# g8a9/multi-modal-emotion

Measured on AMD Instinct MI355X. Metric: utterances/sec fwd+bwd (+clip_grad_norm_+AdamW inside the timed step), TAV (BERT+Wav2Vec2+VideoMAE) b=32, 1/2/4/8 MI355X, higher is better.
Workload: dtype bf16; 1 GPU; tav_nn.py TAV preset B (bert 12 L + wav2vec2 12 L / 768 + videomae 12 L / 768 on 16 frames + fusion 12 L), global batch 32 = 32 per GPU x 1, text 128 tok, audio 80000 samples, video 16x3x224x224 (104 fusion / 1464 encoder tokens), 547.0 GFLOP forward per utterance; global_batch=32, per_gpu_batch=32, parallelism=dp1, weights=random init (seeded), no checkpoints offline, launch=hipGraph replay

## Files before the change

include/tavhip.h:

```cpp
#ifndef TAVHIP_H
#define TAVHIP_H
#include <stdint.h>

#ifdef __cplusplus
extern "C" {
#endif

enum { TAV_F32 = 0, TAV_BF16 = 1, TAV_FP8 = 2  };
enum {
    TAV_ERR_NULL = -1,
    TAV_ERR_SHAPE = -2,
    TAV_ERR_DTYPE = -3,
    TAV_ERR_ALIGN = -4,
    TAV_ERR_NO_RCCL = -5
};

int tav_version(void);
const char* tav_error_string(int code);

typedef struct tav_gemm_nt_args {
    const void* A; const void* B; void* C;
    void* C_pre;
    const float* bias;
    const void* gelu_in;
// ... 20 lines not shown
    float* out;
    float* dbias;
    float* bias_partials;
    int64_t N1, N2;
    int64_t lda, ldb;
    int64_t rows_per_batch, nbatch;
    int64_t a_zb, b_zb;
    int32_t chunk_rows, nsplit;
    int32_t perm_inner, perm_outer;
    int32_t dtype;
    int32_t accumulate;
    float scale;
} tav_gemm_tn_args;
int tav_gemm_tn_splits(int64_t n1, int64_t n2, int64_t rows_per_batch, int64_t nbatch, int32_t* chunk_rows, int32_t* nsplit);
int tav_gemm_tn(const tav_gemm_tn_args* args, void* stream);

typedef struct tav_gemm_tn_problem {
    const void* A; const void* B;
    float* out;
    float* dbias;
    int64_t N1, N2, lda, ldb;
} tav_gemm_tn_problem;
int tav_gemm_tn_grouped(const tav_gemm_tn_problem* problems, int32_t nproblems, int64_t rows, int32_t dtype, void* stream);
int64_t tav_gemm_tn_grouped_ws_bytes(const tav_gemm_tn_problem* problems, int32_t nproblems, int64_t rows, int32_t dtype, int32_t flags);
int tav_gemm_tn_grouped_ws(const tav_gemm_tn_problem* problems, int32_t nproblems, int64_t rows, int32_t dtype, void* workspace,
                           int64_t workspace_bytes, int32_t flags, void* stream);

int tav_fp8_amax_partials(int64_t rows, int64_t cols);
int tav_fp8_amax(const void* x, int32_t dtype, int64_t rows, int64_t cols, int64_t ld, float* partials, float* scales, void* stream);
int tav_fp8_quantize(const void* x, int32_t dtype, int64_t rows, int64_t cols, int64_t ld, const float* scales, void* q, int64_t ld_q, void* qt,
// ... 163 lines not shown
```

multi-modal-emotion_amd/_lib.py:

```python
import ctypes as C
import os

import torch

_HERE = os.path.dirname(os.path.abspath(__file__))
LIB_PATH = os.environ.get("TAV_LIB") or os.path.join(_HERE, "libtavhip.so")

TAV_F32, TAV_BF16, TAV_FP8 = 0, 1, 2
ABI_VERSION = 7

i32, i64, f32, vp = C.c_int32, C.c_int64, C.c_float, C.c_void_p


class GemmNTArgs(C.Structure):
    _fields_ = [("A", vp), ("B", vp), ("C", vp), ("C_pre", vp), ("bias", vp), ("gelu_in", vp), ("resid", vp),
                ("M", i64), ("N", i64), ("K", i64),
                ("lda", i64), ("ldb", i64), ("ldc", i64), ("ld_pre", i64), ("ld_gelu_in", i64), ("ld_resid", i64),
                ("nzb", i32), ("nzg", i32),
                ("a_zb", i64), ("a_zg", i64), ("b_zb", i64), ("b_zg", i64), ("c_zb", i64), ("c_zg", i64), ("bias_zg", i64),
                ("in_dtype", i32), ("out_dtype", i32), ("act", i32), ("accumulate", i32), ("alpha", f32),
                ("a_dequant", vp), ("b_dequant", vp), ("gelu_zb", i64), ("tile_m_hint", i32)]


class GemmTNArgs(C.Structure):
# ... 32 lines not shown


class TextEmbedArgs(C.Structure):
    _fields_ = [("ids", vp), ("word", vp), ("pos", vp), ("type", vp), ("gamma", vp), ("beta", vp), ("pre", vp), ("pos_ids", vp),
                ("y_f32", vp), ("y_lp", vp), ("lp_dtype", i32), ("mean", vp), ("rstd", vp),
                ("B", i64), ("S", i64), ("W", i64), ("vocab", i64), ("max_pos", i64), ("pad_id", i32), ("eps", f32)]


_SIGS = {
    "tav_version": (C.c_int, []),
    "tav_error_string": (C.c_char_p, [C.c_int]),
    "tav_gemm_nt": (C.c_int, [C.POINTER(GemmNTArgs), vp]),
    "tav_gemm_nt_schedule": (C.c_int, [C.POINTER(GemmNTArgs), C.POINTER(i32), C.POINTER(i32), C.POINTER(i32)]),
    "tav_gemm_tn_splits": (C.c_int, [i64, i64, i64, i64, C.POINTER(i32), C.POINTER(i32)]),
    "tav_gemm_tn": (C.c_int, [C.POINTER(GemmTNArgs), vp]),
    "tav_gemm_tn_grouped": (C.c_int, [C.POINTER(GemmTNProblem), i32, i64, i32, vp]),
    "tav_gemm_tn_grouped_ws_bytes": (C.c_int64, [C.POINTER(GemmTNProblem), i32, i64, i32, i32]),
    "tav_gemm_tn_grouped_ws": (C.c_int, [C.POINTER(GemmTNProblem), i32, i64, i32, vp, i64, i32, vp]),
    "tav_colsum": (C.c_int, [vp, i32, i64, i64, i64, vp, i32, vp, i32, vp]),
    "tav_fp8_amax_partials": (C.c_int, [i64, i64]),
    "tav_fp8_amax": (C.c_int, [vp, i32, i64, i64, i64, vp, vp, vp]),
    "tav_fp8_quantize": (C.c_int, [vp, i32, i64, i64, i64, vp, vp, i64, vp, i64, i64, vp]),
    "tav_fp8_quantize_delayed": (C.c_int, [vp, i32, i64, i64, i64, vp, vp, i64, vp, i64, i64, vp]),
    "tav_fp8_roll_states": (C.c_int, [vp, i64, vp]),
    "tav_splitk_reduce": (C.c_int, [vp, vp, i32, i64, i32, vp]),
    "tav_comm_rccl_version": (C.c_int, [C.POINTER(i32)]),
    "tav_comm_unique_id": (C.c_int, [vp]),
    "tav_comm_init_rank": (C.c_int, [C.POINTER(vp), i32, vp, i32]),
    "tav_comm_destroy": (C.c_int, [vp]),
    "tav_allreduce_bucket": (C.c_int, [vp, i64, i32, vp, vp]),
# ... 109 lines not shown
```

multi-modal-emotion_amd/csrc/gemm.hip:

```cpp
#include <stdlib.h>
#include "common.h"
#include <type_traits>
#include "tavhip_internal.h"

namespace tav {

struct GemmNT {
    const char* A; const char* B; char* C; char* Cpre; const float* bias; const char* gelu_in; const float* resid;
    int M, N, K;
    long lda, ldb, ldc, ld_pre, ld_gelu, ld_resid;
    int nzg;
    long a_zb, a_zg, b_zb, b_zg, c_zb, c_zg, bias_zg;
    long g_zb;
    int act, accumulate;
    float alpha;
    int tiles_m, tiles_n;
    const float* sa; const float* sb;
};

TAV_DEV int swz(int row, int chunk) { return chunk ^ ((row >> 1) & 7); }

#ifdef TAV_ABL_NOMFMA
#define TAV_NT_MMA(b, a, c) do { (c)[0] += __uint_as_float((b).x ^ (a).x); } while (0)
#else
// ... 377 lines not shown
        }
    }
}

struct GemmTN {
    const char* A; const char* B; float* S;
    float* bias_part;
    int bias_spread;
    int N1, N2;
    long lda, ldb;
    int rows_per_batch;
    long a_zb, b_zb;
    int chunk_rows;
    int chunks_per_batch;
    int tiles_1, tiles_2;
};

template <typename T> struct TNTile {
    static constexpr int ES = ET<T>::ES, ROWB = 128 * ES, CPR = ROWB / 16;
    static TAV_DEV int sw(int row, int chunk) { return ES == 2 ? (chunk ^ ((row & 7) << 1)) : (chunk ^ (((row >> 2) & 1) << 2)); }
};
template <typename T> TAV_DEV uint4 tn_frag(const char* tile, int krow0, int col0, int lane);
template <> TAV_DEV uint4 tn_frag<bf16>(const char* tile, int krow0, int col0, int lane) {
    using TT = TNTile<bf16>;
    const int g = lane >> 4, i = lane & 15, q = i >> 2, p = i & 3;
    const int r0 = krow0 + 4 * g + q, r1 = r0 + 16;
    const int cb = (col0 + 4 * p) * 2;
    const char* a0 = tile + r0 * TT::ROWB + (TT::sw(r0, cb >> 4) << 4) + (cb & 15);
    const char* a1 = tile + r1 * TT::ROWB + (TT::sw(r1, cb >> 4) << 4) + (cb & 15);
    const uint2 lo = lds_read_tr16(a0), hi = lds_read_tr16(a1);
// ... 37 lines not shown
    constexpr int WROWS = KT / 4;
    constexpr int NINST = WROWS / RPI;
    static_assert(KT % KSTEP == 0 && WROWS % RPI == 0 && NINST >= 1, "TN tile shape");
    extern __shared__ __attribute__((aligned(16))) char smem[];
    char* sA = smem;
    char* sB = smem + NST * TILE_BYTES;

    const int tid = threadIdx.x, lane = tid & 63, wave = tid >> 6;
    const int g = lane >> 4, i = lane & 15;
    const int w1 = wave >> 1, w2 = wave & 1;

    int t1, t2;
    if (p.tiles_1 >= p.tiles_2) { t1 = tile / p.tiles_2; t2 = tile - t1 * p.tiles_2; }
    else { t2 = tile / p.tiles_1; t1 = tile - t2 * p.tiles_1; }
    const int n1_0 = t1 * BT, n2_0 = t2 * BT;
    const int zb = split / p.chunks_per_batch, ck = split - zb * p.chunks_per_batch;
    const int row_begin = ck * p.chunk_rows;
    int row_end = row_begin + p.chunk_rows; row_end = row_end < p.rows_per_batch ? row_end : p.rows_per_batch;

    const char* Ab = p.A + zb * p.a_zb * ES;
    const char* Bb = p.B + zb * p.b_zb * ES;

    const int lrow = lane / CPR, lslot = lane % CPR;
    const int a_cmax = (p.N1 - n1_0) * ES / 16, b_cmax = (p.N2 - n2_0) * ES / 16;

    f32x4 acc[4][4];
#pragma unroll
    for (int a = 0; a < 4; ++a)
#pragma unroll
        for (int b = 0; b < 4; ++b) acc[a][b] = f32x4{0.f, 0.f, 0.f, 0.f};
    const bool do_bias = p.bias_part != nullptr && (p.bias_spread || t2 == 0);
// ... 5 lines not shown
    const int nk = (nrows + KT - 1) / KT;
    const unsigned ldsA = __builtin_amdgcn_readfirstlane(lds_addr(sA) + wave * WROWS * ROWB);
    const unsigned ldsB = __builtin_amdgcn_readfirstlane(lds_addr(sB) + wave * WROWS * ROWB);
    const char* Ab0 = Ab + ((long)row_begin * p.lda + n1_0) * ES;
    const char* Bb0 = Bb + ((long)row_begin * p.ldb + n2_0) * ES;
    unsigned offA[NINST], offB[NINST];
#pragma unroll
    for (int j = 0; j < NINST; ++j) {
        const int trow = wave * WROWS + j * RPI + lrow;
        int ca = TT::sw(trow, lslot); ca = ca < a_cmax ? ca : 0;
        int cb = TT::sw(trow, lslot); cb = cb < b_cmax ? cb : 0;
        offA[j] = (unsigned)(trow * p.lda * ES + ca * 16);
        offB[j] = (unsigned)(trow * p.ldb * ES + cb * 16);
    }
    const unsigned strideA = (unsigned)(KT * p.lda * ES), strideB = (unsigned)(KT * p.ldb * ES);
    auto stage = [&](int kt, int buf) {
        const int base_row = row_begin + kt * KT + wave * WROWS;
        const bool full = (kt + 1) * KT <= nrows;
        if (full) {
            const unsigned ka = kt * strideA, kb = kt * strideB;
#pragma unroll
            for (int j = 0; j < NINST; ++j) {
                glds16_m0(Ab0 + ka, offA[j], ldsA + buf * TILE_BYTES + j * 1024);
                glds16_m0(Bb0 + kb, offB[j], ldsB + buf * TILE_BYTES + j * 1024);
            }
        } else {
#pragma unroll 1
            for (int j = 0; j < NINST; ++j) {
                const int r = j * RPI + lrow;
                const int trow = wave * WROWS + r;
                const int ca = TT::sw(trow, lslot), cb = TT::sw(trow, lslot);
                const bool ok = (kt * KT + trow) < nrows;
                uint4 va = make_uint4(0, 0, 0, 0), vb = va;
                if (ok && ca < a_cmax) va = *reinterpret_cast<const uint4*>(Ab + ((long)(base_row + r) * p.lda + n1_0) * ES + ca * 16);
                if (ok && cb < b_cmax) vb = *reinterpret_cast<const uint4*>(Bb + ((long)(base_row + r) * p.ldb + n2_0) * ES + cb * 16);
                *reinterpret_cast<uint4*>(sA + buf * TILE_BYTES + trow * ROWB + lslot * 16) = va;
                *reinterpret_cast<uint4*>(sB + buf * TILE_BYTES + trow * ROWB + lslot * 16) = vb;
            }
        }
    };
    auto compute = [&](int cur, int kt_now) {
        const char* cA = sA + cur * TILE_BYTES;
        const char* cB = sB + cur * TILE_BYTES;
        const bool bias_now = do_bias && (kt_now % bias_mod) == bias_rem;
#pragma unroll
        for (int s = 0; s < KT / KSTEP; ++s) {
            uint4 f1[4], f2[4];
#pragma unroll
            for (int t = 0; t < 4; ++t) {
                f1[t] = tn_frag<T>(cA, s * KSTEP, w1 * 64 + t * 16, lane);
                f2[t] = tn_frag<T>(cB, s * KSTEP, w2 * 64 + t * 16, lane);
            }
#pragma unroll
            for (int a = 0; a < 4; ++a)
#pragma unroll
                for (int b = 0; b < 4; ++b) mma16<T>(f2[b], f1[a], acc[a][b]);
            if (bias_now) {
                if (w2 == 0) { mma16<T>(ones, f1[0], bacc[0]); mma16<T>(ones, f1[1], bacc[1]); }
                else { mma16<T>(ones, f1[2], bacc[0]); mma16<T>(ones, f1[3], bacc[1]); }
            }
        }
    };

#pragma unroll
    for (int t = 0; t < NST - 1; ++t)
        if (t < nk) stage(t, t);
    int cur = 0, kt = 0;
    for (; kt + NST - 1 < nk; ++kt) {
        asm volatile("s_waitcnt vmcnt(%0)" ::"n"((NST - 2) * 2 * NINST) : "memory");
        __syncthreads();
        stage(kt + NST - 1, cur == 0 ? NST - 1 : cur - 1);
        compute(cur, kt);
        cur = cur + 1 == NST ? 0 : cur + 1;
    }
    for (; kt < nk; ++kt) {
        wait_vmcnt0();
        __syncthreads();
        compute(cur, kt);
        cur = cur + 1 == NST ? 0 : cur + 1;
    }
    __syncthreads();

    if (do_bias && g == 0) {
        const long slot = p.bias_spread ? (long)split * p.tiles_2 + t2 : split;
#pragma unroll
        for (int j = 0; j < 2; ++j) {
            const int n1 = n1_0 + w1 * 64 + (2 * w2 + j) * 16 + i;
            if (n1 < p.N1) p.bias_part[slot * p.N1 + n1] = bacc[j][0];
        }
    }
    float* S = p.S + (long)split * p.N1 * p.N2;
#pragma unroll
    for (int a = 0; a < 4; ++a) {
        const int n1 = n1_0 + w1 * 64 + a * 16 + i;
        if (n1 >= p.N1) continue;
#pragma unroll
        for (int b = 0; b < 4; ++b) {
            const int n2 = n2_0 + w2 * 64 + b * 16 + 4 * g;
            if (n2 >= p.N2) continue;
            st4(S + (long)n1 * p.N2 + n2, acc[a][b]);
        }
    }
}

template <typename T>
__global__ __launch_bounds__(256, 2) void gemm_tn_kernel(const GemmTN p) {
    gemm_tn_body<T>(p, xcd_remap(blockIdx.x, p.tiles_1 * p.tiles_2), blockIdx.y);
}

constexpr int TN_GROUP_MAX = 4;
struct GemmTNGroup {
    GemmTN p[TN_GROUP_MAX];
    int tile_end[TN_GROUP_MAX];
    int n;
};
template <typename T>
__global__ __launch_bounds__(256, 2) void gemm_tn_grouped_kernel(const GemmTNGroup grp) {
    const int t = xcd_remap(blockIdx.x, grp.tile_end[grp.n - 1]);
    int g = 0;
#pragma unroll
    for (int k = 0; k < TN_GROUP_MAX - 1; ++k) g += (k < grp.n - 1 && t >= grp.tile_end[k]) ? 1 : 0;
    const int first = g == 0 ? 0 : grp.tile_end[g - 1];
// ... 203 lines not shown
    if (dbias && gid < N1) {
        float b = 0.f;
        for (int s = 0; s < nsplit; ++s) b += bias_part[(long)s * N1 + gid];
        b *= scale;
        dbias[gid] = accumulate ? dbias[gid] + b : b;
    }
    const long idx4 = gid * 4;
    if (idx4 >= n_elems) return;
    f32x4 v = {0.f, 0.f, 0.f, 0.f};
    for (int s = 0; s < nsplit; ++s) v += ld4(S + (long)s * n_elems + idx4);
    v *= scale;
    if (outer == 1) {
        if (accumulate) v += ld4(out + idx4);
        st4(out + idx4, v);
    } else {
        const long n1 = idx4 / N2; const int n2 = (int)(idx4 - n1 * N2);
#pragma unroll
        for (int e = 0; e < 4; ++e) {
            const int q = n2 + e;
            const long o = n1 * N2 + (long)(q % inner) * outer + q / inner;
            out[o] = accumulate ? out[o] + v[e] : v[e];
        }
    }
}

__global__ void bias_reduce_kernel(const float* __restrict__ part, float* __restrict__ out, int nsplit, int N1, int accumulate, float scale) {
    const int n = blockIdx.x * blockDim.x + threadIdx.x;
    if (n >= N1) return;
    float s = 0.f;
    for (int k = 0; k < nsplit; ++k) s += part[(long)k * N1 + n];
// ... 225 lines not shown
        if (p.gelu_in) q.gelu_in = p.gelu_in + r * p.ld_gelu * es;
        if (p.resid) q.resid = p.resid + r * p.ld_resid;
        p.M = rows_big;
        launch(p, 16);
        launch(q, tm_rest);
    } else {
        launch(p, tm);
    }
#undef TAV_NT_LAUNCH
#undef TAV_NT_LAUNCH_S
    return (int)hipGetLastError();
}

static double split_penalty() { return 0.06; }

extern "C" int tav_gemm_tn_splits(int64_t n1, int64_t n2, int64_t rows_per_batch, int64_t nbatch, int32_t* chunk_rows, int32_t* nsplit) {
    if (!chunk_rows || !nsplit || n1 <= 0 || n2 <= 0 || rows_per_batch <= 0 || nbatch <= 0) return TAV_ERR_SHAPE;
    const long tiles = ((n1 + 127) / 128) * ((n2 + 127) / 128);
    const long SLOTS = 512;
    long best_cpb = 1; double best_score = -1.0;
    const long max_cpb = (rows_per_batch + 255) / 256 > 0 ? (rows_per_batch + 255) / 256 : 1;
    for (long cpb = 1; cpb <= max_cpb && cpb <= 64; ++cpb) {
        long cr = (rows_per_batch + cpb - 1) / cpb;
        cr = ((cr + 63) / 64) * 64;
        const long real_cpb = (rows_per_batch + cr - 1) / cr;
        const long wgs = tiles * real_cpb * nbatch;
        const long rounds = (wgs + SLOTS - 1) / SLOTS;
        double eff = (double)wgs / (double)(rounds * SLOTS);
        const double work = (double)rounds * (double)cr;
        const double ideal = (double)tiles * nbatch * rows_per_batch / SLOTS;
        double score = ideal / work - split_penalty() * (double)(real_cpb * nbatch);
        (void)eff;
        if (score > best_score + 1e-9) { best_score = score; best_cpb = real_cpb; }
    }
    long cr = (rows_per_batch + best_cpb - 1) / best_cpb;
    cr = ((cr + 63) / 64) * 64;
    const long cpb = (rows_per_batch + cr - 1) / cr;
    *chunk_rows = (int32_t)cr;
    *nsplit = (int32_t)(cpb * nbatch);
    return 0;
}

extern "C" int tav_gemm_tn_grouped(const tav_gemm_tn_problem* probs, int32_t nprob, int64_t rows, int32_t dtype, void* stream_) {
    hipStream_t stream = (hipStream_t)stream_;
    if (!probs) return TAV_ERR_NULL;
    if (nprob <= 0 || nprob > TN_GROUP_MAX || rows <= 0) return TAV_ERR_SHAPE;
    if (dtype != TAV_BF16 && dtype != TAV_F32) return TAV_ERR_DTYPE;
    const int es = dtype == TAV_BF16 ? 2 : 4, pk = 16 / es;
    GemmTNGroup grp;
    int total = 0;
    for (int k = 0; k < TN_GROUP_MAX; ++k) {
        const tav_gemm_tn_problem& a = probs[k < nprob ? k : nprob - 1];
        if (k < nprob) {
            if (!a.A || !a.B || !a.out) return TAV_ERR_NULL;
            if (a.N1 <= 0 || a.N2 <= 0) return TAV_ERR_SHAPE;
            if (a.N1 % pk || a.N2 % pk || a.N2 % 4) return TAV_ERR_SHAPE;
            if (a.lda % pk || a.ldb % pk) return TAV_ERR_ALIGN;
            if ((rows + 64) * (a.lda > a.ldb ? a.lda : a.ldb) * es >= (1ll << 32)) return TAV_ERR_SHAPE;
        }
        GemmTN& p = grp.p[k];
        p.A = (const char*)a.A; p.B = (const char*)a.B; p.S = a.out; p.bias_part = a.dbias; p.bias_spread = 0;
        p.N1 = (int)a.N1; p.N2 = (int)a.N2; p.lda = a.lda; p.ldb = a.ldb;
        p.rows_per_batch = (int)rows; p.a_zb = 0; p.b_zb = 0;
        p.chunk_rows = (int)(((rows + 63) / 64) * 64); p.chunks_per_batch = 1;
        p.tiles_1 = (p.N1 + 127) / 128; p.tiles_2 = (p.N2 + 127) / 128;
        if (k < nprob) total += p.tiles_1 * p.tiles_2;
        grp.tile_end[k] = total;
    }
    grp.n = nprob;
    dim3 grid(total), block(256);
    if (dtype == TAV_BF16) hipLaunchKernelGGL((gemm_tn_grouped_kernel<bf16>), grid, block, 4 * 64 * 256, stream, grp);
    else hipLaunchKernelGGL((gemm_tn_grouped_kernel<float>), grid, block, 4 * 64 * 512, stream, grp);
    return (int)hipGetLastError();
}

static bool tn_big_plan(const tav_gemm_tn_problem* probs, int nprob, long rows, int dtype, int flags, int* nsplit, long* ws_floats) {
    *nsplit = 1; *ws_floats = 0;
    const bool can_big = dtype == TAV_BF16 && !(flags & 2);
    long tiles = 0, elems = 0;
// ... 45 lines not shown
    bool any_bias = false;
    const long chunk = ((rows + nsplit - 1) / nsplit + 63) / 64 * 64;
    if ((long)(nsplit - 1) * chunk >= rows) return TAV_ERR_SHAPE;
    float* ws = (float*)workspace;
    long ws_off = 0, end4 = 0;
    for (int k = 0; k < TN_GROUP_MAX; ++k) {
        const tav_gemm_tn_problem& a = probs[k < nprob ? k : nprob - 1];
        if (k < nprob) {
            if (!a.A || !a.B || !a.out) return TAV_ERR_NULL;
            if (a.N1 <= 0 || a.N2 <= 0 || a.N1 % pk || a.N2 % pk || a.N2 % 4) return TAV_ERR_SHAPE;
            if (a.lda % pk || a.ldb % pk) return TAV_ERR_ALIGN;
            if ((rows + 64) * (a.lda > a.ldb ? a.lda : a.ldb) * es >= (1ll << 32)) return TAV_ERR_SHAPE;
        }
        GemmTN& p = grp.p[k];
        p.A = (const char*)a.A; p.B = (const char*)a.B; p.N1 = (int)a.N1; p.N2 = (int)a.N2; p.lda = a.lda; p.ldb = a.ldb;
        p.rows_per_batch = (int)rows; p.a_zb = 0; p.b_zb = 0; p.chunk_rows = (int)chunk; p.chunks_per_batch = nsplit;
        p.tiles_1 = (p.N1 + tw - 1) / tw; p.tiles_2 = (p.N2 + tw - 1) / tw;
        if (nsplit > 1) { p.S = ws + ws_off; if (k < nprob) ws_off += (long)nsplit * a.N1 * a.N2; }
        else p.S = a.out;
        p.bias_part = nullptr; p.bias_spread = 1;
        if (k < nprob) total += p.tiles_1 * p.tiles_2;
        grp.tile_end[k] = total;
        red.slabs[k] = p.S; red.out[k] = a.out; red.dbias[k] = a.dbias; red.N1[k] = (int)a.N1; red.n4[k] = a.N1 * a.N2 / 4;
        red.nbias[k] = nsplit * p.tiles_2; red.bias_part[k] = nullptr;
        if (k < nprob) { end4 += red.n4[k]; total_n1 += (int)a.N1; any_bias |= a.dbias != nullptr; }
        red.end4[k] = end4;
    }
    for (int k = 0; k < nprob; ++k) {
        if (!probs[k].dbias) continue;
        grp.p[k].bias_part = ws + ws_off; red.bias_part[k] = ws + ws_off;
        ws_off += (long)red.nbias[k] * probs[k].N1;
    }
    grp.n = nprob; red.n = nprob; red.nsplit = nsplit;
    if (big) hipLaunchKernelGGL((gemm_tn_grouped_big_kernel<bf16>), dim3(total, nsplit), dim3(512), (TAV_TN_RING25 ? 5 : 4) * 2 * 64 * 256, stream, grp);
    else if (dtype == TAV_BF16) hipLaunchKernelGGL((gemm_tn_grouped_kernel<bf16>), dim3(total), dim3(256), 4 * 64 * 256, stream, grp);
    else hipLaunchKernelGGL((gemm_tn_grouped_kernel<float>), dim3(total), dim3(256), 4 * 64 * 512, stream, grp);
    if (nsplit > 1) hipLaunchKernelGGL(tn_group_reduce_kernel, dim3((unsigned)((end4 + 255) / 256)), dim3(256), 0, stream, red);
    else if (any_bias) hipLaunchKernelGGL(tn_group_bias_reduce_kernel, dim3((unsigned)((total_n1 + 255) / 256)), dim3(256), 0, stream, red, total_n1);
    return (int)hipGetLastError();
}

extern "C" int tav_gemm_tn(const tav_gemm_tn_args* a, void* stream_) {
    hipStream_t stream = (hipStream_t)stream_;
    if (!a || !a->A || !a->B || !a->slabs || !a->out) return TAV_ERR_NULL;
    if (a->N1 <= 0 || a->N2 <= 0 || a->rows_per_batch <= 0 || a->nbatch <= 0) return TAV_ERR_SHAPE;
    if (a->dtype != TAV_BF16 && a->dtype != TAV_F32) return TAV_ERR_DTYPE;
    const int es = a->dtype == TAV_BF16 ? 2 : 4, pk = 16 / es;
    if (a->N1 % pk || a->N2 % pk || a->N2 % 4) return TAV_ERR_SHAPE;
    if (a->lda % pk || a->ldb % pk || a->a_zb % pk || a->b_zb % pk) return TAV_ERR_ALIGN;
    if (a->chunk_rows <= 0 || a->chunk_rows % 64) return TAV_ERR_SHAPE;
    if ((a->rows_per_batch + 64) * (a->lda > a->ldb ? a->lda : a->ldb) * es >= (1ll << 32)) return TAV_ERR_SHAPE;
    GemmTN p;
    p.A = (const char*)a->A; p.B = (const char*)a->B; p.S = a->slabs;
    p.bias_part = a->dbias ? a->bias_partials : nullptr; p.bias_spread = 0;
    if (a->dbias && !a->bias_partials) return TAV_ERR_NULL;
    p.N1 = (int)a->N1; p.N2 = (int)a->N2; p.lda = a->lda; p.ldb = a->ldb;
    p.rows_per_batch = (int)a->rows_per_batch; p.a_zb = a->a_zb; p.b_zb = a->b_zb;
    p.chunk_rows = a->chunk_rows;
    p.chunks_per_batch = (int)((a->rows_per_batch + a->chunk_rows - 1) / a->chunk_rows);
    const int nsplit = p.chunks_per_batch * (int)a->nbatch;
    if (nsplit != a->nsplit) return TAV_ERR_SHAPE;
    p.tiles_1 = (p.N1 + 127) / 128; p.tiles_2 = (p.N2 + 127) / 128;
    const int inner = a->perm_inner > 0 ? a->perm_inner : p.N2, outer = a->perm_outer > 0 ? a->perm_outer : 1;
    if (outer > 1 && inner * outer != p.N2) return TAV_ERR_SHAPE;
    dim3 grid(p.tiles_1 * p.tiles_2, nsplit), block(256);
    if (a->dtype == TAV_BF16) {
        const size_t lds = 4 * 64 * 256;
        hipLaunchKernelGGL((gemm_tn_kernel<bf16>), grid, block, lds, stream, p);
    } else {
        const size_t lds = 4 * 64 * 512;
        hipLaunchKernelGGL((gemm_tn_kernel<float>), grid, block, lds, stream, p);
    }
    int e = (int)hipGetLastError();
    if (e) return e;
    const long n_elems = (long)p.N1 * p.N2;
    const long nthreads = (n_elems + 3) / 4;
    hipLaunchKernelGGL(splitk_reduce_kernel, dim3((unsigned)((nthreads + 255) / 256)), dim3(256), 0, stream, a->slabs, a->out, nsplit,
                       n_elems, p.N2, inner, outer, a->accumulate, a->scale == 0.f ? 1.f : a->scale, (const float*)a->bias_partials, a->dbias, p.N1);
    return (int)hipGetLastError();
}

extern "C" int tav_colsum(const void* x, int32_t dtype, int64_t M, int64_t N, int64_t ld, float* partials, int32_t nparts, float* out,
                          int32_t accumulate, void* stream_) {
    hipStream_t stream = (hipStream_t)stream_;
    if (!x || !partials || !out) return TAV_ERR_NULL;
    if (M <= 0 || N <= 0 || nparts <= 0) return TAV_ERR_SHAPE;
    const int rows_per_block = (int)((M + nparts - 1) / nparts);
    dim3 grid((unsigned)((N + 255) / 256), nparts), block(256);
    if (dtype == TAV_BF16) hipLaunchKernelGGL((colsum_partial_kernel<bf16>), grid, block, 0, stream, (const bf16*)x, partials, (int)M, (int)N, (long)ld, rows_per_block);
    else if (dtype == TAV_F32) hipLaunchKernelGGL((colsum_partial_kernel<float>), grid, block, 0, stream, (const float*)x, partials, (int)M, (int)N, (long)ld, rows_per_block);
    else return TAV_ERR_DTYPE;
    hipLaunchKernelGGL(colsum_final_kernel, dim3((unsigned)((N + 255) / 256)), dim3(256), 0, stream, partials, out, nparts, (int)N, accumulate);
    return (int)hipGetLastError();
// ... 2 lines not shown
```

multi-modal-emotion_amd/engine.py:

```python
import os
import weakref

import torch

from . import ops

_EPOCH = [0]


def bump_weight_epoch():
    _EPOCH[0] += 1


class Policy:
    def __init__(self, name="bf16"):
        name = {"bfloat16": "bf16", "float32": "fp32", "f32": "fp32", "float8": "fp8", "e4m3": "fp8"}.get(name, name)
        if name not in ("bf16", "fp32", "fp8", "fp8-all", "fp8-wgrad8"):
            raise ValueError(f"unknown precision policy {name!r}")
        self.name = name
        self.lp = torch.float32 if name == "fp32" else torch.bfloat16
        self.f32 = name == "fp32"
        self.fp8 = name.startswith("fp8")
        self.fp8_stacks = () if not self.fp8 else (("video", "text", "audio", "fusion") if name == "fp8-all" else ("video",))
        self.fp8_wgrad8 = name in ("fp8-wgrad8", "fp8-all")
# ... 770 lines not shown
    @staticmethod
    def backward(ctx, gout):
        xg, pre, v, g, norms = ctx.saved_tensors
        pol = ctx.ectx.pol
        B, T, H, G, Cg, K = ctx.geom
        gout = _c(gout)
        _, wf, _ = ctx.ectx.cache.posconv(v, g)
        du = ops.gelu_bwd(pre, gout)
        pad = K // 2
        dug = ops.group_pad(du, B, T, H, G, pad - 1, pad, pol.lp)
        TPd, TP = T + 2 * pad - 1, T + 2 * pad
        dx = ops.gemm_nt(dug, wf, resid=gout, out_dtype=torch.float32, M=T, N=Cg, K=K * Cg, lda=Cg, ldb=K * Cg, ldc=H, nzb=B, nzg=G,
                         a_zb=G * TPd * Cg, a_zg=TPd * Cg, b_zg=Cg * K * Cg, c_zb=T * H, c_zg=Cg, out_shape=(B * T, H))
        du_lp = _to_lp(pol, du)
        dw = torch.empty(G, Cg, K * Cg, dtype=torch.float32, device=du.device)
        for gi in range(G):
            ops.gemm_tn(du_lp[:, gi * Cg:], xg[:, gi], out=dw[gi], N1=Cg, N2=K * Cg, lda=H, ldb=Cg, rows_per_batch=T, nbatch=B, a_zb=T * H,
                        b_zb=G * TP * Cg)
        dv, dg = ops.weight_norm_bwd(v, g, norms, dw)
        dbias = ops.colsum(du)
        return dx, dv, dg.view_as(g), dbias, None, None, None, None


class ConcatSeqFn(torch.autograd.Function):

    @staticmethod
    def forward(ctx, B, *parts):
        W = parts[0].shape[-1]
        lens = [p.numel() // (B * W) for p in parts]
        Sf = sum(lens)
        out = torch.empty(B, Sf, W, dtype=torch.float32, device=parts[0].device)
        flat = out.view(B, Sf * W)
        off = 0
# ... 207 lines not shown
```

multi-modal-emotion_amd/ops.py:

```python
import ctypes as C
import os

import torch

from . import _lib as L
from ._lib import check, dt, lib, ptr, stream

_ws = {}


def workspace(name, nfloats, device):
    key = (name, torch.cuda.current_stream().cuda_stream, str(device))
    t = _ws.get(key)
    if t is None or t.numel() < nfloats:
        t = torch.empty(max(int(nfloats), 1), dtype=torch.float32, device=device)
        _ws[key] = t
    return t


def clear_workspaces():
    _ws.clear()


_prof = None
# ... 93 lines not shown
    g.rows_per_batch, g.nbatch, g.a_zb, g.b_zb = rows_per_batch, nbatch, a_zb, b_zb
    g.chunk_rows, g.nsplit, g.perm_inner, g.perm_outer = cr.value, ns.value, perm_inner, perm_outer
    g.dtype, g.accumulate, g.scale = dt(a), int(accumulate), scale
    dbias = None
    if want_bias:
        dbias = torch.empty(N1, dtype=torch.float32, device=a.device)
        bpart = workspace("tn_bias", ns.value * N1, a.device)
        g.dbias, g.bias_partials = ptr(dbias), ptr(bpart)
    assert a.dtype == b.dtype
    tokens = rows_per_batch * nbatch
    _prof_launch("gemm_tn", "bf16" if a.dtype == torch.bfloat16 else "f32", 2.0 * tokens * N1 * N2, tokens * (N1 + N2) * a.element_size() + 4 * N1 * N2,
                 lambda: check(lib().tav_gemm_tn(C.byref(g), stream()), "gemm_tn"))
    return (out, dbias) if want_bias else out


def gemm_tn_grouped(pairs, want_bias=True, flags=0, into=None):
    n = len(pairs)
    rows, dtype = pairs[0][0].shape[0], pairs[0][0].dtype
    probs = (L.GemmTNProblem * n)()
    outs = []
    for k, (a, b) in enumerate(pairs):
        assert a.shape[0] == rows and b.shape[0] == rows and a.dtype == dtype and b.dtype == dtype
        N1, N2 = a.shape[1], b.shape[1]
        dW_to, db_to = into[k] if into is not None else (None, None)
        dW = dW_to if dW_to is not None else torch.empty(N1, N2, dtype=torch.float32, device=a.device)
        db = (db_to if db_to is not None else torch.empty(N1, dtype=torch.float32, device=a.device)) if want_bias else None
        assert dW.shape == (N1, N2) and dW.is_contiguous() and dW.dtype == torch.float32 and (db is None or (db.shape == (N1,) and db.is_contiguous()))
        pr = probs[k]
        pr.A, pr.B, pr.out, pr.dbias = ptr(a), ptr(b), ptr(dW), ptr(db)
        pr.N1, pr.N2, pr.lda, pr.ldb = N1, N2, a.stride(0), b.stride(0)
# ... 570 lines not shown
```

Measured before the change: 420.5 utterances/s.

## Batch grouped-conv weight-grad GEMMs into one multi-problem launch with batch-per-item splits

Replaces the per-group loop of gemm_tn launches in the wav2vec2 positional grouped-conv backward with a single multi-problem TN GEMM kernel that handles up to 16 groups, plus a fused split-K reduce across all problems. The split planner can now assign several batch entries to one workgroup (batch_per_item), cutting the number of fp32 partial slabs and reduce traffic. It also rewrites the partial-tile staging path to use a register-buffered unrolled load. The cost is full vmcnt waits in the multi path, extra accumulator registers for per-entry flushing in bf16, and a larger slab workspace.

```diff
diff --git a/include/tavhip.h b/include/tavhip.h
--- a/include/tavhip.h
+++ b/include/tavhip.h
@@ -58,6 +58,9 @@
 } tav_gemm_tn_args;
 int tav_gemm_tn_splits(int64_t n1, int64_t n2, int64_t rows_per_batch, int64_t nbatch, int32_t* chunk_rows, int32_t* nsplit);
 int tav_gemm_tn(const tav_gemm_tn_args* args, void* stream);
+int tav_gemm_tn_multi_splits(int64_t n1, int64_t n2, int64_t rows_per_batch, int64_t nbatch, int32_t nproblems, int32_t* chunk_rows,
+                             int32_t* nsplit);
+int tav_gemm_tn_multi(const tav_gemm_tn_args* args, int32_t nargs, void* stream);
 
 typedef struct tav_gemm_tn_problem {
     const void* A; const void* B;
diff --git a/multi-modal-emotion_amd/_lib.py b/multi-modal-emotion_amd/_lib.py
--- a/multi-modal-emotion_amd/_lib.py
+++ b/multi-modal-emotion_amd/_lib.py
@@ -70,6 +70,8 @@
     "tav_gemm_nt_schedule": (C.c_int, [C.POINTER(GemmNTArgs), C.POINTER(i32), C.POINTER(i32), C.POINTER(i32)]),
     "tav_gemm_tn_splits": (C.c_int, [i64, i64, i64, i64, C.POINTER(i32), C.POINTER(i32)]),
     "tav_gemm_tn": (C.c_int, [C.POINTER(GemmTNArgs), vp]),
+    "tav_gemm_tn_multi_splits": (C.c_int, [i64, i64, i64, i64, i32, C.POINTER(i32), C.POINTER(i32)]),
+    "tav_gemm_tn_multi": (C.c_int, [C.POINTER(GemmTNArgs), i32, vp]),
     "tav_gemm_tn_grouped": (C.c_int, [C.POINTER(GemmTNProblem), i32, i64, i32, vp]),
     "tav_gemm_tn_grouped_ws_bytes": (C.c_int64, [C.POINTER(GemmTNProblem), i32, i64, i32, i32]),
     "tav_gemm_tn_grouped_ws": (C.c_int, [C.POINTER(GemmTNProblem), i32, i64, i32, vp, i64, i32, vp]),
diff --git a/multi-modal-emotion_amd/csrc/gemm.hip b/multi-modal-emotion_amd/csrc/gemm.hip
--- a/multi-modal-emotion_amd/csrc/gemm.hip
+++ b/multi-modal-emotion_amd/csrc/gemm.hip
@@ -415,6 +415,8 @@
     int chunk_rows;
     int chunks_per_batch;
     int tiles_1, tiles_2;
+    int batch_per_item;
+    int nbatch;
 };
 
 template <typename T> struct TNTile {
@@ -482,7 +484,9 @@
     if (p.tiles_1 >= p.tiles_2) { t1 = tile / p.tiles_2; t2 = tile - t1 * p.tiles_2; }
     else { t2 = tile / p.tiles_1; t1 = tile - t2 * p.tiles_1; }
     const int n1_0 = t1 * BT, n2_0 = t2 * BT;
-    const int zb = split / p.chunks_per_batch, ck = split - zb * p.chunks_per_batch;
+    const bool multi = p.batch_per_item > 1;
+    const int zb = multi ? split * p.batch_per_item : split / p.chunks_per_batch, ck = multi ? 0 : split - zb * p.chunks_per_batch;
+    const int nb = multi ? (p.nbatch - zb < p.batch_per_item ? p.nbatch - zb : p.batch_per_item) : 1;
     const int row_begin = ck * p.chunk_rows;
     int row_end = row_begin + p.chunk_rows; row_end = row_end < p.rows_per_batch ? row_end : p.rows_per_batch;
 
@@ -518,30 +522,38 @@
         offB[j] = (unsigned)(trow * p.ldb * ES + cb * 16);
     }
     const unsigned strideA = (unsigned)(KT * p.lda * ES), strideB = (unsigned)(KT * p.ldb * ES);
-    auto stage = [&](int kt, int buf) {
-        const int base_row = row_begin + kt * KT + wave * WROWS;
+    int s_kt = 0;
+    const char* s_A = Ab0;
+    const char* s_B = Bb0;
+    auto stage = [&](int buf) {
+        const int kt = s_kt;
         const bool full = (kt + 1) * KT <= nrows;
         if (full) {
             const unsigned ka = kt * strideA, kb = kt * strideB;
 #pragma unroll
             for (int j = 0; j < NINST; ++j) {
-                glds16_m0(Ab0 + ka, offA[j], ldsA + buf * TILE_BYTES + j * 1024);
-                glds16_m0(Bb0 + kb, offB[j], ldsB + buf * TILE_BYTES + j * 1024);
+                glds16_m0(s_A + ka, offA[j], ldsA + buf * TILE_BYTES + j * 1024);
+                glds16_m0(s_B + kb, offB[j], ldsB + buf * TILE_BYTES + j * 1024);
             }
         } else {
-#pragma unroll 1
+            uint4 va[NINST], vb[NINST];
+#pragma unroll
             for (int j = 0; j < NINST; ++j) {
-                const int r = j * RPI + lrow;
-                const int trow = wave * WROWS + r;
+                const int trow = wave * WROWS + j * RPI + lrow;
                 const int ca = TT::sw(trow, lslot), cb = TT::sw(trow, lslot);
                 const bool ok = (kt * KT + trow) < nrows;
-                uint4 va = make_uint4(0, 0, 0, 0), vb = va;
-                if (ok && ca < a_cmax) va = *reinterpret_cast<const uint4*>(Ab + ((long)(base_row + r) * p.lda + n1_0) * ES + ca * 16);
-                if (ok && cb < b_cmax) vb = *reinterpret_cast<const uint4*>(Bb + ((long)(base_row + r) * p.ldb + n2_0) * ES + cb * 16);
-                *reinterpret_cast<uint4*>(sA + buf * TILE_BYTES + trow * ROWB + lslot * 16) = va;
-                *reinterpret_cast<uint4*>(sB + buf * TILE_BYTES + trow * ROWB + lslot * 16) = vb;
-            }
-        }
+                va[j] = make_uint4(0, 0, 0, 0); vb[j] = va[j];
+                if (ok && ca < a_cmax) va[j] = *reinterpret_cast<const uint4*>(s_A + (long)(kt * KT + trow) * p.lda * ES + ca * 16);
+                if (ok && cb < b_cmax) vb[j] = *reinterpret_cast<const uint4*>(s_B + (long)(kt * KT + trow) * p.ldb * ES + cb * 16);
+            }
+#pragma unroll
+            for (int j = 0; j < NINST; ++j) {
+                const int trow = wave * WROWS + j * RPI + lrow;
+                *reinterpret_cast<uint4*>(sA + buf * TILE_BYTES + trow * ROWB + lslot * 16) = va[j];
+                *reinterpret_cast<uint4*>(sB + buf * TILE_BYTES + trow * ROWB + lslot * 16) = vb[j];
+            }
+        }
+        if (++s_kt == nk) { s_kt = 0; s_A += p.a_zb * ES; s_B += p.b_zb * ES; }
     };
     auto compute = [&](int cur, int kt_now) {
         const char* cA = sA + cur * TILE_BYTES;
@@ -566,24 +578,52 @@
         }
     };
 
+    const int nq = nb * nk;
 #pragma unroll
     for (int t = 0; t < NST - 1; ++t)
-        if (t < nk) stage(t, t);
+        if (t < nq) stage(t);
     int cur = 0, kt = 0;
-    for (; kt + NST - 1 < nk; ++kt) {
-        asm volatile("s_waitcnt vmcnt(%0)" ::"n"((NST - 2) * 2 * NINST) : "memory");
+    constexpr bool FLUSH = ES == 2;
+    f32x4 tot[4][4], btot[2] = {f32x4{0.f, 0.f, 0.f, 0.f}, f32x4{0.f, 0.f, 0.f, 0.f}};
+#pragma unroll
+    for (int a = 0; a < 4; ++a)
+#pragma unroll
+        for (int b = 0; b < 4; ++b) tot[a][b] = f32x4{0.f, 0.f, 0.f, 0.f};
+    int e_kt = 0;
+    auto entry_end = [&]() {
+        if (!FLUSH || !multi || ++e_kt < nk) return;
+        e_kt = 0;
+#pragma unroll
+        for (int a = 0; a < 4; ++a)
+#pragma unroll
+            for (int b = 0; b < 4; ++b) { tot[a][b] += acc[a][b]; acc[a][b] = f32x4{0.f, 0.f, 0.f, 0.f}; }
+#pragma unroll
+        for (int j = 0; j < 2; ++j) { btot[j] += bacc[j]; bacc[j] = f32x4{0.f, 0.f, 0.f, 0.f}; }
+    };
+    for (; kt + NST - 1 < nq; ++kt) {
+        if (NST == 2 || multi) wait_vmcnt0();
+        else asm volatile("s_waitcnt vmcnt(%0)" ::"n"((NST - 2) * 2 * NINST) : "memory");
         __syncthreads();
-        stage(kt + NST - 1, cur == 0 ? NST - 1 : cur - 1);
+        stage(cur == 0 ? NST - 1 : cur - 1);
         compute(cur, kt);
+        entry_end();
         cur = cur + 1 == NST ? 0 : cur + 1;
     }
-    for (; kt < nk; ++kt) {
+    for (; kt < nq; ++kt) {
         wait_vmcnt0();
         __syncthreads();
         compute(cur, kt);
+        entry_end();
         cur = cur + 1 == NST ? 0 : cur + 1;
     }
     __syncthreads();
+    if (FLUSH && multi) {
+#pragma unroll
+        for (int a = 0; a < 4; ++a)
+#pragma unroll
+            for (int b = 0; b < 4; ++b) acc[a][b] = tot[a][b];
+        bacc[0] = btot[0]; bacc[1] = btot[1];
+    }
 
     if (do_bias && g == 0) {
         const long slot = p.bias_spread ? (long)split * p.tiles_2 + t2 : split;
@@ -610,6 +650,24 @@
 template <typename T>
 __global__ __launch_bounds__(256, 2) void gemm_tn_kernel(const GemmTN p) {
     gemm_tn_body<T>(p, xcd_remap(blockIdx.x, p.tiles_1 * p.tiles_2), blockIdx.y);
+}
+
+constexpr int TN_MULTI_MAX = 16;
+struct GemmTNMulti {
+    GemmTN p[TN_MULTI_MAX];
+    int item_end[TN_MULTI_MAX];
+    int n;
+};
+template <typename T>
+__global__ __launch_bounds__(256, 2) void gemm_tn_multi_kernel(const GemmTNMulti m) {
+    const int it = xcd_remap(blockIdx.x, m.item_end[m.n - 1]);
+    int g = 0;
+#pragma unroll
+    for (int k = 0; k < TN_MULTI_MAX - 1; ++k) g += (k < m.n - 1 && it >= m.item_end[k]) ? 1 : 0;
+    const int local = it - (g == 0 ? 0 : m.item_end[g - 1]);
+    const int tiles = m.p[g].tiles_1 * m.p[g].tiles_2;
+    const int split = local / tiles;
+    gemm_tn_body<T>(m.p[g], local - split * tiles, split);
 }
 
 constexpr int TN_GROUP_MAX = 4;
@@ -843,6 +901,50 @@
         if (accumulate) v += ld4(out + idx4);
         st4(out + idx4, v);
     } else {
+        const long n1 = idx4 / N2; const int n2 = (int)(idx4 - n1 * N2);
+#pragma unroll
+        for (int e = 0; e < 4; ++e) {
+            const int q = n2 + e;
+            const long o = n1 * N2 + (long)(q % inner) * outer + q / inner;
+            out[o] = accumulate ? out[o] + v[e] : v[e];
+        }
+    }
+}
+
+struct TNMultiReduce {
+    const float* slabs[TN_MULTI_MAX]; float* out[TN_MULTI_MAX]; const float* bias_part[TN_MULTI_MAX]; float* dbias[TN_MULTI_MAX];
+    long end4[TN_MULTI_MAX];
+    int N1[TN_MULTI_MAX], N2[TN_MULTI_MAX], nsplit[TN_MULTI_MAX], inner[TN_MULTI_MAX], outer[TN_MULTI_MAX], accumulate[TN_MULTI_MAX];
+    float scale[TN_MULTI_MAX];
+    int n;
+};
+__global__ void tn_multi_reduce_kernel(const TNMultiReduce r) {
+    const long g0 = (long)blockIdx.x * blockDim.x + threadIdx.x;
+    if (g0 >= r.end4[r.n - 1]) return;
+    int k = 0;
+#pragma unroll
+    for (int q = 0; q < TN_MULTI_MAX - 1; ++q) k += (q < r.n - 1 && g0 >= r.end4[q]) ? 1 : 0;
+    const long gid = g0 - (k == 0 ? 0 : r.end4[k - 1]);
+    const int nsplit = r.nsplit[k], N1 = r.N1[k], N2 = r.N2[k], accumulate = r.accumulate[k];
+    const float scale = r.scale[k];
+    const long n_elems = (long)N1 * N2;
+    float* out = r.out[k];
+    if (r.dbias[k] && gid < N1) {
+        float b = 0.f;
+        for (int s = 0; s < nsplit; ++s) b += r.bias_part[k][(long)s * N1 + gid];
+        b *= scale;
+        r.dbias[k][gid] = accumulate ? r.dbias[k][gid] + b : b;
+    }
+    const long idx4 = gid * 4;
+    if (idx4 >= n_elems) return;
+    f32x4 v = {0.f, 0.f, 0.f, 0.f};
+    for (int s = 0; s < nsplit; ++s) v += ld4(r.slabs[k] + (long)s * n_elems + idx4);
+    v *= scale;
+    if (r.outer[k] == 1) {
+        if (accumulate) v += ld4(out + idx4);
+        st4(out + idx4, v);
+    } else {
+        const int inner = r.inner[k], outer = r.outer[k];
         const long n1 = idx4 / N2; const int n2 = (int)(idx4 - n1 * N2);
 #pragma unroll
         for (int e = 0; e < 4; ++e) {
@@ -1098,30 +1200,46 @@
 
 static double split_penalty() { return 0.06; }
 
-extern "C" int tav_gemm_tn_splits(int64_t n1, int64_t n2, int64_t rows_per_batch, int64_t nbatch, int32_t* chunk_rows, int32_t* nsplit) {
-    if (!chunk_rows || !nsplit || n1 <= 0 || n2 <= 0 || rows_per_batch <= 0 || nbatch <= 0) return TAV_ERR_SHAPE;
-    const long tiles = ((n1 + 127) / 128) * ((n2 + 127) / 128);
+static void tn_plan(long tiles, long rows_per_batch, long nbatch, int32_t* chunk_rows, int32_t* nsplit) {
     const long SLOTS = 512;
-    long best_cpb = 1; double best_score = -1.0;
+    long best_cpb = 1, best_bpi = 1; double best_score = -1e30;
     const long max_cpb = (rows_per_batch + 255) / 256 > 0 ? (rows_per_batch + 255) / 256 : 1;
+    const double ideal = (double)tiles * nbatch * rows_per_batch / SLOTS;
     for (long cpb = 1; cpb <= max_cpb && cpb <= 64; ++cpb) {
         long cr = (rows_per_batch + cpb - 1) / cpb;
         cr = ((cr + 63) / 64) * 64;
         const long real_cpb = (rows_per_batch + cr - 1) / cr;
         const long wgs = tiles * real_cpb * nbatch;
         const long rounds = (wgs + SLOTS - 1) / SLOTS;
-        double eff = (double)wgs / (double)(rounds * SLOTS);
         const double work = (double)rounds * (double)cr;
-        const double ideal = (double)tiles * nbatch * rows_per_batch / SLOTS;
-        double score = ideal / work - split_penalty() * (double)(real_cpb * nbatch);
-        (void)eff;
-        if (score > best_score + 1e-9) { best_score = score; best_cpb = real_cpb; }
+        const double score = ideal / work - split_penalty() * (double)(real_cpb * nbatch);
+        if (score > best_score + 1e-9) { best_score = score; best_cpb = real_cpb; best_bpi = 1; }
+    }
+    const long cr1 = ((rows_per_batch + 63) / 64) * 64;
+    for (long bpi = 2; bpi <= nbatch && bpi * cr1 <= 2048; ++bpi) {
+        const long ns = (nbatch + bpi - 1) / bpi;
+        if ((nbatch + ns - 1) / ns != bpi) continue;
+        const long wgs = tiles * ns;
+        const long rounds = (wgs + SLOTS - 1) / SLOTS;
+        const double work = (double)rounds * (double)(cr1 * bpi);
+        const double score = ideal / work - split_penalty() * (double)ns;
+        if (score > best_score + 1e-9) { best_score = score; best_cpb = 1; best_bpi = bpi; }
     }
     long cr = (rows_per_batch + best_cpb - 1) / best_cpb;
     cr = ((cr + 63) / 64) * 64;
     const long cpb = (rows_per_batch + cr - 1) / cr;
     *chunk_rows = (int32_t)cr;
-    *nsplit = (int32_t)(cpb * nbatch);
+    *nsplit = (int32_t)(best_bpi > 1 ? (nbatch + best_bpi - 1) / best_bpi : cpb * nbatch);
+}
+
+extern "C" int tav_gemm_tn_splits(int64_t n1, int64_t n2, int64_t rows_per_batch, int64_t nbatch, int32_t* chunk_rows, int32_t* nsplit) {
+    return tav_gemm_tn_multi_splits(n1, n2, rows_per_batch, nbatch, 1, chunk_rows, nsplit);
+}
+
+extern "C" int tav_gemm_tn_multi_splits(int64_t n1, int64_t n2, int64_t rows_per_batch, int64_t nbatch, int32_t nproblems, int32_t* chunk_rows,
+                                        int32_t* nsplit) {
+    if (!chunk_rows || !nsplit || n1 <= 0 || n2 <= 0 || rows_per_batch <= 0 || nbatch <= 0 || nproblems <= 0 || nproblems > TN_MULTI_MAX) return TAV_ERR_SHAPE;
+    tn_plan(((n1 + 127) / 128) * ((n2 + 127) / 128) * nproblems, rows_per_batch, nbatch, chunk_rows, nsplit);
     return 0;
 }
 
@@ -1146,7 +1264,7 @@
         p.A = (const char*)a.A; p.B = (const char*)a.B; p.S = a.out; p.bias_part = a.dbias; p.bias_spread = 0;
         p.N1 = (int)a.N1; p.N2 = (int)a.N2; p.lda = a.lda; p.ldb = a.ldb;
         p.rows_per_batch = (int)rows; p.a_zb = 0; p.b_zb = 0;
-        p.chunk_rows = (int)(((rows + 63) / 64) * 64); p.chunks_per_batch = 1;
+        p.chunk_rows = (int)(((rows + 63) / 64) * 64); p.chunks_per_batch = 1; p.batch_per_item = 1; p.nbatch = 1;
         p.tiles_1 = (p.N1 + 127) / 128; p.tiles_2 = (p.N2 + 127) / 128;
         if (k < nprob) total += p.tiles_1 * p.tiles_2;
         grp.tile_end[k] = total;
@@ -1222,7 +1340,7 @@
         }
         GemmTN& p = grp.p[k];
         p.A = (const char*)a.A; p.B = (const char*)a.B; p.N1 = (int)a.N1; p.N2 = (int)a.N2; p.lda = a.lda; p.ldb = a.ldb;
-        p.rows_per_batch = (int)rows; p.a_zb = 0; p.b_zb = 0; p.chunk_rows = (int)chunk; p.chunks_per_batch = nsplit;
+        p.rows_per_batch = (int)rows; p.a_zb = 0; p.b_zb = 0; p.chunk_rows = (int)chunk; p.chunks_per_batch = nsplit; p.batch_per_item = 1; p.nbatch = 1;
         p.tiles_1 = (p.N1 + tw - 1) / tw; p.tiles_2 = (p.N2 + tw - 1) / tw;
         if (nsplit > 1) { p.S = ws + ws_off; if (k < nprob) ws_off += (long)nsplit * a.N1 * a.N2; }
         else p.S = a.out;
@@ -1248,9 +1366,8 @@
     return (int)hipGetLastError();
 }
 
-extern "C" int tav_gemm_tn(const tav_gemm_tn_args* a, void* stream_) {
-    hipStream_t stream = (hipStream_t)stream_;
-    if (!a || !a->A || !a->B || !a->slabs || !a->out) return TAV_ERR_NULL;
+static int tn_fill(const tav_gemm_tn_args* a, GemmTN& p, int& nsplit) {
+    if (!a->A || !a->B || !a->slabs || !a->out) return TAV_ERR_NULL;
     if (a->N1 <= 0 || a->N2 <= 0 || a->rows_per_batch <= 0 || a->nbatch <= 0) return TAV_ERR_SHAPE;
     if (a->dtype != TAV_BF16 && a->dtype != TAV_F32) return TAV_ERR_DTYPE;
     const int es = a->dtype == TAV_BF16 ? 2 : 4, pk = 16 / es;
@@ -1258,7 +1375,6 @@
     if (a->lda % pk || a->ldb % pk || a->a_zb % pk || a->b_zb % pk) return TAV_ERR_ALIGN;
     if (a->chunk_rows <= 0 || a->chunk_rows % 64) return TAV_ERR_SHAPE;
     if ((a->rows_per_batch + 64) * (a->lda > a->ldb ? a->lda : a->ldb) * es >= (1ll << 32)) return TAV_ERR_SHAPE;
-    GemmTN p;
     p.A = (const char*)a->A; p.B = (const char*)a->B; p.S = a->slabs;
     p.bias_part = a->dbias ? a->bias_partials : nullptr; p.bias_spread = 0;
     if (a->dbias && !a->bias_partials) return TAV_ERR_NULL;
@@ -1266,11 +1382,27 @@
     p.rows_per_batch = (int)a->rows_per_batch; p.a_zb = a->a_zb; p.b_zb = a->b_zb;
     p.chunk_rows = a->chunk_rows;
     p.chunks_per_batch = (int)((a->rows_per_batch + a->chunk_rows - 1) / a->chunk_rows);
-    const int nsplit = p.chunks_per_batch * (int)a->nbatch;
+    p.nbatch = (int)a->nbatch; p.batch_per_item = 1;
+    nsplit = p.chunks_per_batch * (int)a->nbatch;
+    if (p.chunks_per_batch == 1 && a->nsplit > 0 && a->nsplit < a->nbatch) {
+        p.batch_per_item = (int)((a->nbatch + a->nsplit - 1) / a->nsplit);
+        nsplit = (int)((a->nbatch + p.batch_per_item - 1) / p.batch_per_item);
+    }
     if (nsplit != a->nsplit) return TAV_ERR_SHAPE;
     p.tiles_1 = (p.N1 + 127) / 128; p.tiles_2 = (p.N2 + 127) / 128;
     const int inner = a->perm_inner > 0 ? a->perm_inner : p.N2, outer = a->perm_outer > 0 ? a->perm_outer : 1;
     if (outer > 1 && inner * outer != p.N2) return TAV_ERR_SHAPE;
+    return 0;
+}
+
+extern "C" int tav_gemm_tn(const tav_gemm_tn_args* a, void* stream_) {
+    hipStream_t stream = (hipStream_t)stream_;
+    if (!a) return TAV_ERR_NULL;
+    GemmTN p;
+    int nsplit;
+    const int rc = tn_fill(a, p, nsplit);
+    if (rc) return rc;
+    const int inner = a->perm_inner > 0 ? a->perm_inner : p.N2, outer = a->perm_outer > 0 ? a->perm_outer : 1;
     dim3 grid(p.tiles_1 * p.tiles_2, nsplit), block(256);
     if (a->dtype == TAV_BF16) {
         const size_t lds = 4 * 64 * 256;
@@ -1285,6 +1417,37 @@
     const long nthreads = (n_elems + 3) / 4;
     hipLaunchKernelGGL(splitk_reduce_kernel, dim3((unsigned)((nthreads + 255) / 256)), dim3(256), 0, stream, a->slabs, a->out, nsplit,
                        n_elems, p.N2, inner, outer, a->accumulate, a->scale == 0.f ? 1.f : a->scale, (const float*)a->bias_partials, a->dbias, p.N1);
+    return (int)hipGetLastError();
+}
+
+extern "C" int tav_gemm_tn_multi(const tav_gemm_tn_args* args, int32_t nargs, void* stream_) {
+    hipStream_t stream = (hipStream_t)stream_;
+    if (!args) return TAV_ERR_NULL;
+    if (nargs <= 0 || nargs > TN_MULTI_MAX) return TAV_ERR_SHAPE;
+    GemmTNMulti m;
+    TNMultiReduce r;
+    int items = 0;
+    long end4 = 0;
+    for (int k = 0; k < TN_MULTI_MAX; ++k) {
+        const tav_gemm_tn_args* a = &args[k < nargs ? k : nargs - 1];
+        if (a->dtype != args[0].dtype) return TAV_ERR_DTYPE;
+        int nsplit;
+        const int rc = tn_fill(a, m.p[k], nsplit);
+        if (rc) return rc;
+        const GemmTN& p = m.p[k];
+        if (k < nargs) { items += p.tiles_1 * p.tiles_2 * nsplit; end4 += ((long)p.N1 * p.N2 + 3) / 4; }
+        m.item_end[k] = items;
+        r.slabs[k] = a->slabs; r.out[k] = a->out; r.bias_part[k] = (const float*)a->bias_partials; r.dbias[k] = a->dbias;
+        r.end4[k] = end4; r.N1[k] = p.N1; r.N2[k] = p.N2; r.nsplit[k] = nsplit;
+        r.inner[k] = a->perm_inner > 0 ? a->perm_inner : p.N2; r.outer[k] = a->perm_outer > 0 ? a->perm_outer : 1;
+        r.accumulate[k] = a->accumulate; r.scale[k] = a->scale == 0.f ? 1.f : a->scale;
+    }
+    m.n = nargs; r.n = nargs;
+    if (args[0].dtype == TAV_BF16) hipLaunchKernelGGL((gemm_tn_multi_kernel<bf16>), dim3(items), dim3(256), 4 * 64 * 256, stream, m);
+    else hipLaunchKernelGGL((gemm_tn_multi_kernel<float>), dim3(items), dim3(256), 4 * 64 * 512, stream, m);
+    int e = (int)hipGetLastError();
+    if (e) return e;
+    hipLaunchKernelGGL(tn_multi_reduce_kernel, dim3((unsigned)((end4 + 255) / 256)), dim3(256), 0, stream, r);
     return (int)hipGetLastError();
 }
 
diff --git a/multi-modal-emotion_amd/engine.py b/multi-modal-emotion_amd/engine.py
--- a/multi-modal-emotion_amd/engine.py
+++ b/multi-modal-emotion_amd/engine.py
@@ -808,9 +808,10 @@
                          a_zb=G * TPd * Cg, a_zg=TPd * Cg, b_zg=Cg * K * Cg, c_zb=T * H, c_zg=Cg, out_shape=(B * T, H))
         du_lp = _to_lp(pol, du)
         dw = torch.empty(G, Cg, K * Cg, dtype=torch.float32, device=du.device)
-        for gi in range(G):
-            ops.gemm_tn(du_lp[:, gi * Cg:], xg[:, gi], out=dw[gi], N1=Cg, N2=K * Cg, lda=H, ldb=Cg, rows_per_batch=T, nbatch=B, a_zb=T * H,
-                        b_zb=G * TP * Cg)
+        for g0 in range(0, G, 16):
+            gis = range(g0, min(g0 + 16, G))
+            ops.gemm_tn_multi([du_lp[:, gi * Cg:] for gi in gis], [xg[:, gi] for gi in gis], [dw[gi] for gi in gis], N1=Cg, N2=K * Cg, lda=H, ldb=Cg,
+                              rows_per_batch=T, nbatch=B, a_zb=T * H, b_zb=G * TP * Cg)
         dv, dg = ops.weight_norm_bwd(v, g, norms, dw)
         dbias = ops.colsum(du)
         return dx, dv, dg.view_as(g), dbias, None, None, None, None
diff --git a/multi-modal-emotion_amd/ops.py b/multi-modal-emotion_amd/ops.py
--- a/multi-modal-emotion_amd/ops.py
+++ b/multi-modal-emotion_amd/ops.py
@@ -131,6 +131,27 @@
     return (out, dbias) if want_bias else out
 
 
+def gemm_tn_multi(a_list, b_list, outs, *, N1, N2, lda, ldb, rows_per_batch, nbatch=1, a_zb=0, b_zb=0, perm_inner=0, perm_outer=0):
+    n = len(a_list)
+    assert 0 < n <= 16 and len(b_list) == n and len(outs) == n
+    cr, ns = C.c_int32(), C.c_int32()
+    check(lib().tav_gemm_tn_multi_splits(N1, N2, rows_per_batch, nbatch, n, C.byref(cr), C.byref(ns)), "gemm_tn_multi_splits")
+    slabs = workspace("tn_slabs", n * ns.value * N1 * N2, a_list[0].device)
+    gs = (L.GemmTNArgs * n)()
+    for k, (a, b, out) in enumerate(zip(a_list, b_list, outs)):
+        assert a.dtype == b.dtype == a_list[0].dtype and out.dtype == torch.float32 and out.is_contiguous() and out.numel() == N1 * N2
+        g = gs[k]
+        g.A, g.B, g.slabs, g.out = ptr(a), ptr(b), slabs.data_ptr() + 4 * k * ns.value * N1 * N2, ptr(out)
+        g.N1, g.N2, g.lda, g.ldb = N1, N2, lda, ldb
+        g.rows_per_batch, g.nbatch, g.a_zb, g.b_zb = rows_per_batch, nbatch, a_zb, b_zb
+        g.chunk_rows, g.nsplit, g.perm_inner, g.perm_outer = cr.value, ns.value, perm_inner, perm_outer
+        g.dtype, g.accumulate, g.scale = dt(a), 0, 1.0
+    tokens = rows_per_batch * nbatch
+    _prof_launch("gemm_tn", "bf16" if a_list[0].dtype == torch.bfloat16 else "f32", 2.0 * tokens * N1 * N2 * n,
+                 n * (tokens * (N1 + N2) * a_list[0].element_size() + 4 * N1 * N2), lambda: check(lib().tav_gemm_tn_multi(gs, n, stream()), "gemm_tn_multi"))
+    return outs
+
+
 def gemm_tn_grouped(pairs, want_bias=True, flags=0, into=None):
     n = len(pairs)
     rows, dtype = pairs[0][0].shape[0], pairs[0][0].dtype
```

Result: no change. 420.6 utterances/s, median of 5 (+0.0%).
